# usnistgov/alignn

Measured on NVIDIA H100. Metric: graphs/sec fwd+bwd, higher is better.
Workload: dtype f32

## Files before the change

### alignn_b200/_lib.py

```python
from __future__ import annotations

import ctypes as C
import os
from typing import Optional

import torch

_HERE = os.path.dirname(os.path.abspath(__file__))
LIB_PATH = os.path.join(_HERE, "libalignn_b200.so")

NORM_LAYER, NORM_AFFINE, NORM_STATS = 0, 1, 2
SUPPORTED_D = (32, 64, 128, 256)

_fp = C.c_void_p


class EgcFwdArgs(C.Structure):
    _fields_ = [
        ("struct_size", C.c_size_t),
        ("Nn", C.c_int64), ("Ne", C.c_int64),
        ("d", C.c_int32), ("norm_nodes", C.c_int32), ("norm_edges", C.c_int32), ("residual", C.c_int32),
        ("gate_is_m", C.c_int32),
        ("gate_eps", C.c_float), ("ln_eps", C.c_float),
        ("x", _fp), ("y", _fp), ("G", _fp), ("P", _fp),
        ("src", _fp), ("in_ptr", _fp), ("in_eid", _fp),
        ("n_w", _fp), ("n_b", _fp), ("e_w", _fp), ("e_b", _fp),
        ("x_out", _fp), ("y_out", _fp), ("M", _fp), ("XP", _fp), ("S", _fp), ("H", _fp),
        ("partials", _fp),
        ("stream", _fp),
    ]


class EgcBwdArgs(C.Structure):
    _fields_ = [
        ("struct_size", C.c_size_t),
        ("Nn", C.c_int64), ("Ne", C.c_int64),
        ("d", C.c_int32), ("norm_nodes", C.c_int32), ("norm_edges", C.c_int32),
        ("gate_eps", C.c_float), ("ln_eps", C.c_float),
        ("P", _fp), ("M", _fp), ("XP", _fp), ("S", _fp), ("H", _fp),
        ("src", _fp), ("dst", _fp), ("in_ptr", _fp), ("in_eid", _fp), ("out_ptr", _fp), ("out_eid", _fp),
        ("n_w", _fp), ("n_b", _fp), ("n_mean", _fp), ("n_rstd", _fp),
        ("e_w", _fp), ("e_b", _fp), ("e_mean", _fp), ("e_rstd", _fp),
        ("n_c1", _fp), ("n_c2", _fp), ("e_c1", _fp), ("e_c2", _fp),
        ("gx_out", _fp), ("gy_out", _fp),
        ("GM", _fp), ("GP", _fp), ("GSh", _fp),
        ("partials", _fp), ("partials_src", _fp),
        ("stream", _fp),
    ]


class EgcBwdVjpArgs(C.Structure):
    _fields_ = [
        ("struct_size", C.c_size_t),
        ("Nn", C.c_int64), ("Ne", C.c_int64),
        ("d", C.c_int32), ("norm", C.c_int32),
        ("gate_eps", C.c_float), ("ln_eps", C.c_float),
        ("P", _fp), ("M", _fp), ("XP", _fp), ("S", _fp), ("H", _fp),
        ("src", _fp), ("dst", _fp), ("in_ptr", _fp), ("in_eid", _fp), ("out_ptr", _fp), ("out_eid", _fp),
        ("n_w", _fp), ("n_b", _fp), ("e_w", _fp), ("e_b", _fp),
        ("gx_out", _fp), ("gy_out", _fp), ("GSh", _fp),
        ("GPbar", _fp), ("GMbar", _fp), ("gx_bar_res", _fp), ("gy_bar_res", _fp),
        ("Pbar", _fp), ("Mbar", _fp), ("gx_out_bar", _fp), ("gy_out_bar", _fp), ("Gamma", _fp), ("Shbar", _fp),
        ("partials", _fp), ("partials_src", _fp),
        ("stream", _fp),
    ]


class GemmGatherArgs(C.Structure):
    _fields_ = [
        ("struct_size", C.c_size_t),
        ("M", C.c_int64), ("N", C.c_int32), ("K", C.c_int32),
        ("A", _fp), ("lda", C.c_int64),
        ("w_image", _fp), ("bias", _fp),
        ("add0", _fp), ("ld0", C.c_int64), ("idx0", _fp),
        ("add1", _fp), ("ld1", C.c_int64), ("idx1", _fp),
        ("C", _fp), ("ldc", C.c_int64),
        ("stats", _fp),
        ("stream", _fp),
    ]
# ... 133 lines not shown
```

### alignn_b200/csrc/egc_kernels.cu

```cuda
#include "common.cuh"
#include "api_common.h"
#include "alignn_b200.h"

namespace alignn {

template <int D, bool GIM>
__global__ void __launch_bounds__(kThreads, 2)
egc_forward_kernel(alignn_b200_egc_fwd_args a) {
  using C = RowCfg<D>;
  constexpr int V = C::VPL;
  extern __shared__ __align__(16) float dyn_smem[];
  float* vec = dyn_smem;
  float* sacc = dyn_smem + 4 * D;
  const int lane = threadIdx.x & 31, wib = threadIdx.x >> 5;
  const int64_t warp0 = (int64_t)blockIdx.x * kWarpsPerBlock + wib;
  const int64_t nwarps = (int64_t)gridDim.x * kWarpsPerBlock;
  const bool train = a.XP != nullptr;
  const bool want_res = a.residual && a.y_out && a.norm_edges != ALIGNN_NORM_STATS;
  const bool stats = a.partials != nullptr;
  {
    const float* srcs[4] = {a.n_w, a.n_b, a.e_w, a.e_b};
#pragma unroll
    for (int q = 0; q < 4; ++q)
      for (int i = threadIdx.x; i < D; i += blockDim.x) vec[q * D + i] = srcs[q] ? srcs[q][i] : 0.f;
// ... 369 lines not shown
#pragma unroll
    for (int k = 0; k < V; ++k) t1[k] *= xh[k];
    smem_row_add<D>(acc_gw, t1, lane);
    sa = warp_sum(sa) * (1.f / D);
    sb = warp_sum(sb) * (1.f / D);
#pragma unroll
    for (int k = 0; k < V; ++k) gr[k] = rstd * (gxh[k] - sa - xh[k] * sb);
  } else {
    float mu[V], rs[V], t0[V], t1[V];
    ld_srow<D>(mu, vecs + 2 * D, lane);
    ld_srow<D>(rs, vecs + 3 * D, lane);
#pragma unroll
    for (int k = 0; k < V; ++k) {
      const float gu = go[k] * dsilu_(r[k] * w[k] + b[k]);
      const float xh = (r[k] - mu[k]) * rs[k];
      t0[k] = gu * xh;
      t1[k] = gu;
      gr[k] = w[k] * gu;
      mu[k] = xh;
    }
    smem_row_add<D>(acc_gw, t0, lane);
    smem_row_add<D>(acc_gb, t1, lane);
    if constexpr (mode == ALIGNN_NORM_STATS) {
      float c1[V], c2[V];
      ld_srow<D>(c1, vecs + 4 * D, lane);
      ld_srow<D>(c2, vecs + 5 * D, lane);
#pragma unroll
      for (int k = 0; k < V; ++k) gr[k] -= w[k] * (c1[k] + mu[k] * c2[k]);
    }
  }
}

template <int D, int NORM>
__global__ void __launch_bounds__(kThreads)
egc_backward_dst_kernel(alignn_b200_egc_bwd_args a) {
  using C = RowCfg<D>;
  constexpr int V = C::VPL;
  extern __shared__ __align__(16) float dyn_smem[];
  float* sacc = dyn_smem;
  float* nvec = dyn_smem + kWarpsPerBlock * 6 * D;
  float* sseg = nvec + 12 * D;
  float* evec = nvec + 6 * D;
  {
    const float* srcs[12] = {a.n_w, a.n_b, a.n_mean, a.n_rstd, a.n_c1, a.n_c2, a.e_w, a.e_b, a.e_mean, a.e_rstd, a.e_c1, a.e_c2};
#pragma unroll
    for (int q = 0; q < 12; ++q)
      for (int i = threadIdx.x; i < D; i += blockDim.x) nvec[q * D + i] = srcs[q] ? srcs[q][i] : 0.f;
  }
  __syncthreads();
  const int lane = threadIdx.x & 31, wib = threadIdx.x >> 5;
  const int64_t warp0 = (int64_t)blockIdx.x * kWarpsPerBlock + wib;
  const int64_t nwarps = (int64_t)gridDim.x * kWarpsPerBlock;
  float* acc = sacc + wib * 6 * D;
  for (int i = lane; i < 6 * D; i += 32) acc[i] = 0.f;
  __syncwarp();

  float* wseg = sseg + wib * 2 * D;
  for (int64_t v = warp0; v < a.Nn; v += nwarps) {
    {
      float gsh[V], gs[V];
      float xp[V], go[V], gxp[V], sv[V], hv[V];
      ld_row<D, false>(xp, a.XP + v * D, lane);
      ld_row<D, false>(go, a.gx_out + v * D, lane);
      norm_backward_row<D, NORM>(xp, go, a.ln_eps, nvec, gxp, acc + 2 * D, acc + 3 * D, lane);
      st_row<D, false>(a.GP + v * 4 * D + 3 * D, gxp, lane);
      ld_row<D, false>(sv, a.S + v * D, lane);
      ld_row<D, false>(hv, a.H + v * D, lane);
#pragma unroll
      for (int k = 0; k < V; ++k) {
        const float inv = 1.f / (sv[k] + a.gate_eps);
        gsh[k] = gxp[k] * inv;
        gs[k] = -gxp[k] * hv[k] * inv;
      }
      smem_row_add<D>(acc + 4 * D, gxp, lane);
      st_row<D, false>(a.GSh + v * D, gsh, lane);
      using C2 = RowCfg<D>;
#pragma unroll
      for (int c = 0; c < C2::CH; ++c)
#pragma unroll
        for (int j = 0; j < C2::W; ++j) {
          wseg[c * 32 * C2::W + lane * C2::W + j] = gsh[c * C2::W + j];
          wseg[D + c * 32 * C2::W + lane * C2::W + j] = gs[c * C2::W + j];
        }
      __syncwarp();
    }
    float accB[V];
#pragma unroll
    for (int k = 0; k < V; ++k) accB[k] = 0.f;
    const int p0 = a.in_ptr[v], p1 = a.in_ptr[v + 1];
    for (int base = p0; base < p1; base += 32) {
      const int cnt = min(32, p1 - base);
      int my_e = 0, my_s = 0;
      if (lane < cnt) {
        my_e = a.in_eid ? a.in_eid[base + lane] : base + lane;
        my_s = a.src[my_e];
      }
      float m[V], go[V];
      if (cnt > 0) {
        const int64_t e = __shfl_sync(0xffffffffu, my_e, 0);
        ld_row<D, true>(m, a.M + e * D, lane);
        if (a.gy_out) ld_row<D, true>(go, a.gy_out + e * D, lane);
      }
      for (int i = 0; i < cnt; ++i) {
        const int64_t e = __shfl_sync(0xffffffffu, my_e, i);
        const int64_t s = __shfl_sync(0xffffffffu, my_s, i);
        float cv[V], gm[V], mn[V], gon[V];
        ld_row<D, false>(cv, a.P + s * 4 * D + D, lane);
        const bool more = (i + 1 < cnt);
        if (more) {
          const int64_t en = __shfl_sync(0xffffffffu, my_e, i + 1);
          ld_row<D, true>(mn, a.M + en * D, lane);
          if (a.gy_out) ld_row<D, true>(gon, a.gy_out + en * D, lane);
        }
        if (a.gy_out) {
          norm_backward_row<D, NORM>(m, go, a.ln_eps, evec, gm, acc, acc + D, lane);
        } else {
#pragma unroll
          for (int k = 0; k < V; ++k) gm[k] = 0.f;
        }
        {
          float gsh[V], gs[V];
          ld_srow<D>(gsh, wseg, lane);
          ld_srow<D>(gs, wseg + D, lane);
#pragma unroll
          for (int k = 0; k < V; ++k) {
            const float sg = sigmoidf_(m[k]);
            gm[k] += (gsh[k] * cv[k] + gs[k]) * sg * (1.f - sg);
            accB[k] += gm[k];
          }
        }
        st_row<D, false>(a.GM + e * D, gm, lane);
        if (more) {
#pragma unroll
          for (int k = 0; k < V; ++k) { m[k] = mn[k]; go[k] = gon[k]; }
        }
      }
    }
    st_row<D, false>(a.GP + v * 4 * D + 2 * D, accB, lane);
    smem_row_add<D>(acc + 5 * D, accB, lane);
  }
  __syncthreads();
  if (a.partials) {
    float* out_row = a.partials + (int64_t)blockIdx.x * 6 * D;
    for (int i = threadIdx.x; i < 6 * D; i += blockDim.x) {
      float t = 0.f;
#pragma unroll
      for (int w = 0; w < kWarpsPerBlock; ++w) t += sacc[w * 6 * D + i];
      out_row[i] = t;
    }
  }
}

template <int D>
__global__ void __launch_bounds__(kThreads)
egc_backward_src_kernel(alignn_b200_egc_bwd_args a, float* __restrict__ partials_src, int partial_rows_total) {
  using C = RowCfg<D>;
  constexpr int V = C::VPL;
  __shared__ float red[kWarpsPerBlock * D];
  const int lane = threadIdx.x & 31;
  const int64_t warp0 = (int64_t)blockIdx.x * kWarpsPerBlock + (threadIdx.x >> 5);
  const int64_t nwarps = (int64_t)gridDim.x * kWarpsPerBlock;
  float acc[2][V];
#pragma unroll
  for (int q = 0; q < 2; ++q)
#pragma unroll
    for (int i = 0; i < V; ++i) acc[q][i] = 0.f;

  for (int64_t u = warp0; u < a.Nn; u += nwarps) {
    float accA[V], accC[V];
#pragma unroll
    for (int k = 0; k < V; ++k) { accA[k] = 0.f; accC[k] = 0.f; }
    const int p0 = a.out_ptr[u], p1 = a.out_ptr[u + 1];
    for (int base = p0; base < p1; base += 32) {
      const int cnt = min(32, p1 - base);
      int my_e = 0, my_t = 0;
      if (lane < cnt) {
        my_e = a.out_eid[base + lane];
        my_t = a.dst[my_e];
      }
      int i = 0;
      for (; i + 1 < cnt; i += 2) {
        const int64_t e0 = __shfl_sync(0xffffffffu, my_e, i), t0 = __shfl_sync(0xffffffffu, my_t, i);
        const int64_t e1 = __shfl_sync(0xffffffffu, my_e, i + 1), t1 = __shfl_sync(0xffffffffu, my_t, i + 1);
        float gm0[V], m0[V], gs0[V], gm1[V], m1[V], gs1[V];
        ld_row<D, false>(gm0, a.GM + e0 * D, lane);
        ld_row<D, false>(gm1, a.GM + e1 * D, lane);
        ld_row<D, true>(m0, a.M + e0 * D, lane);
        ld_row<D, true>(m1, a.M + e1 * D, lane);
        ld_row<D, false>(gs0, a.GSh + t0 * D, lane);
        ld_row<D, false>(gs1, a.GSh + t1 * D, lane);
#pragma unroll
        for (int k = 0; k < V; ++k) { accA[k] += gm0[k]; accC[k] += gs0[k] * sigmoidf_(m0[k]); }
#pragma unroll
        for (int k = 0; k < V; ++k) { accA[k] += gm1[k]; accC[k] += gs1[k] * sigmoidf_(m1[k]); }
      }
      if (i < cnt) {
        const int64_t e = __shfl_sync(0xffffffffu, my_e, i);
        const int64_t t = __shfl_sync(0xffffffffu, my_t, i);
        float gm[V], m[V], gsh[V];
        ld_row<D, false>(gm, a.GM + e * D, lane);
        ld_row<D, true>(m, a.M + e * D, lane);
        ld_row<D, false>(gsh, a.GSh + t * D, lane);
#pragma unroll
        for (int k = 0; k < V; ++k) {
          accA[k] += gm[k];
          accC[k] += gsh[k] * sigmoidf_(m[k]);
        }
      }
    }
    st_row<D, false>(a.GP + u * 4 * D, accA, lane);
    st_row<D, false>(a.GP + u * 4 * D + D, accC, lane);
#pragma unroll
    for (int k = 0; k < V; ++k) { acc[0][k] += accA[k]; acc[1][k] += accC[k]; }
  }
  if (partials_src) {
    block_reduce_to_partials<D, 2>(acc, partials_src + (int64_t)blockIdx.x * 2 * D, red);
    const int extra = blockIdx.x + gridDim.x;
    if (extra < partial_rows_total)
      for (int i = threadIdx.x; i < 2 * D; i += blockDim.x) partials_src[(int64_t)extra * 2 * D + i] = 0.f;
  }
}

__global__ void __launch_bounds__(1024)
bn_finalize_kernel(const float* __restrict__ partials, int rows, int stride, int which, double count,
                   int d, const float* __restrict__ gamma, const float* __restrict__ beta, float eps,
                   float momentum, float* running_mean, float* running_var, float* scale, float* shift,
                   float* mean_out, float* rstd_out) {
  __shared__ double ss[32][33], sq[32][33];
  const int cl = threadIdx.x & 31, rl = threadIdx.x >> 5;
  const int c = blockIdx.x * 32 + cl;
  double s = 0.0, q = 0.0;
  if (c < d) {
    const float* p = partials + (size_t)which * 2 * d + c;
    for (int r = rl; r < rows; r += 32) {
      s += (double)p[(size_t)r * stride];
      q += (double)p[(size_t)r * stride + d];
    }
  }
  ss[rl][cl] = s; sq[rl][cl] = q;
  __syncthreads();
  if (rl != 0 || c >= d) return;
#pragma unroll
  for (int k = 1; k < 32; ++k) { s += ss[k][cl]; q += sq[k][cl]; }
  const double mean = s / count;
  double var = q / count - mean * mean;
  if (var < 0.0) var = 0.0;
  const float rstd = (float)(1.0 / sqrt(var + (double)eps));
  const float g = gamma ? gamma[c] : 1.f, b = beta ? beta[c] : 0.f;
  scale[c] = g * rstd;
  shift[c] = b - (float)mean * g * rstd;
  mean_out[c] = (float)mean;
  rstd_out[c] = rstd;
// ... 396 lines not shown
}

int alignn_b200_affine_silu_residual(const float* R, const float* res, const float* scale, const float* shift, float* out,
                                     int64_t n, int d, alignn_stream_t stream) {
  if (!supported_d(d)) return ALIGNN_ERR_UNSUPPORTED_D;
  if (n < 0 || (n > 0 && (!R || !scale || !shift || !out))) return ALIGNN_ERR_BAD_ARG;
  if (n == 0) return ALIGNN_OK;
  const int grid = grid_for_rows(n);
  DISPATCH_D(d, alignn::affine_silu_residual_kernel<D><<<grid, alignn::kThreads, 0, (cudaStream_t)stream>>>(
                    R, res, scale, shift, out, n));
  return check_launch();
}

int alignn_b200_egc_backward(const alignn_b200_egc_bwd_args* a) {
  if (!a) return ALIGNN_ERR_BAD_ARG;
  if (a->struct_size != sizeof(*a)) return ALIGNN_ERR_STRUCT_SIZE;
  if (!supported_d(a->d)) return ALIGNN_ERR_UNSUPPORTED_D;
  if (a->Nn < 0 || a->Ne < 0 || !norm_ok(a->norm_nodes) || !norm_ok(a->norm_edges)) return ALIGNN_ERR_BAD_ARG;
  if (a->Nn == 0) return ALIGNN_OK;
  if (!a->P || !a->XP || !a->S || !a->H || !a->in_ptr || !a->out_ptr || !a->gx_out || !a->GP || !a->GSh ||
      !a->n_w || !a->n_b)
    return ALIGNN_ERR_BAD_ARG;
  if (a->Ne > 0 && (!a->M || !a->src || !a->dst || !a->out_eid || !a->GM)) return ALIGNN_ERR_BAD_ARG;
  if (a->norm_nodes != ALIGNN_NORM_LAYER && (!a->n_mean || !a->n_rstd)) return ALIGNN_ERR_BAD_ARG;
  if (a->norm_nodes == ALIGNN_NORM_STATS && (!a->n_c1 || !a->n_c2)) return ALIGNN_ERR_BAD_ARG;
  if (a->gy_out) {
    if (!a->e_w || !a->e_b) return ALIGNN_ERR_BAD_ARG;
    if (a->norm_edges != ALIGNN_NORM_LAYER && (!a->e_mean || !a->e_rstd)) return ALIGNN_ERR_BAD_ARG;
    if (a->norm_edges == ALIGNN_NORM_STATS && (!a->e_c1 || !a->e_c2)) return ALIGNN_ERR_BAD_ARG;
  }
  cudaStream_t st = (cudaStream_t)a->stream;
  const int grid = grid_for_rows(a->Nn);
  if (a->norm_nodes != a->norm_edges) return ALIGNN_ERR_BAD_ARG;
#define LAUNCH_BWD_DST(NORM)                                                                                   \
  DISPATCH_D(a->d, {                                                                                           \
    const size_t smem_bytes = (size_t)(alignn::kWarpsPerBlock * 8 + 12) * D * sizeof(float);                   \
    static alignn::DeviceOnce configured; int cfg_dev;                                                                            \
    if (configured.needed(&cfg_dev)) {                                                                                         \
      cudaError_t e = cudaFuncSetAttribute(alignn::egc_backward_dst_kernel<D, NORM>,                           \
                                           cudaFuncAttributeMaxDynamicSharedMemorySize, (int)smem_bytes);      \
      if (e != cudaSuccess) return alignn::record_cuda_error((int)e);                                          \
      configured.done(cfg_dev);                                                                                       \
    }                                                                                                          \
    alignn::egc_backward_dst_kernel<D, NORM><<<grid, alignn::kThreads, smem_bytes, st>>>(*a);                  \
  })
  switch (a->norm_nodes) {
    case ALIGNN_NORM_LAYER: LAUNCH_BWD_DST(ALIGNN_NORM_LAYER); break;
    case ALIGNN_NORM_AFFINE: LAUNCH_BWD_DST(ALIGNN_NORM_AFFINE); break;
    default: LAUNCH_BWD_DST(ALIGNN_NORM_STATS); break;
  }
#undef LAUNCH_BWD_DST
  int rc = check_launch();
  if (rc != ALIGNN_OK) return rc;
  DISPATCH_D(a->d, {
    const int grid_src = alignn::one_wave_grid((const void*)alignn::egc_backward_src_kernel<D>, alignn::kThreads, 0, grid);
    if (2 * grid_src < grid) return ALIGNN_ERR_CUDA;
    alignn::egc_backward_src_kernel<D><<<grid_src, alignn::kThreads, 0, st>>>(*a, a->partials_src, grid);
  });
  return check_launch();
}

int alignn_b200_bn_backward_reduce(const float* R, const float* g_out, const float* scale, const float* shift,
                                   const float* mean, const float* rstd, int64_t n, int d, float* partials,
                                   int partial_rows, alignn_stream_t stream) {
  if (!supported_d(d)) return ALIGNN_ERR_UNSUPPORTED_D;
  if (n <= 0 || !R || !g_out || !scale || !shift || !mean || !rstd || !partials) return ALIGNN_ERR_BAD_ARG;
// ... 98 lines not shown
```

### alignn_b200/graph.py

```python
from __future__ import annotations

from typing import Optional, Sequence

import numpy as np
import torch

__all__ = ["Graph", "EdgeIndex", "batch", "unbatch", "reverse", "graph", "as_graph", "bond_cosines"]


def _np(a):
    if isinstance(a, torch.Tensor):
        return a.detach().cpu().numpy()
    return np.asarray(a)


class EdgeIndex:

    __slots__ = ("src", "dst", "in_ptr", "in_eid", "out_ptr", "out_eid", "dst_sorted",
                 "max_in_deg", "num_nodes")

    def __init__(self, src, dst, in_ptr, in_eid, out_ptr, out_eid, dst_sorted, max_in_deg, num_nodes):
        self.src, self.dst = src, dst
        self.in_ptr, self.in_eid = in_ptr, in_eid
        self.out_ptr, self.out_eid = out_ptr, out_eid
        self.dst_sorted = bool(dst_sorted)
        self.max_in_deg = int(max_in_deg)
        self.num_nodes = int(num_nodes)

    @staticmethod
    def build(src: np.ndarray, dst: np.ndarray, num_nodes: int) -> "EdgeIndex":
        from . import _lib
        lib = _lib.load()
        src = np.ascontiguousarray(src, dtype=np.int64).reshape(-1)
        dst = np.ascontiguousarray(dst, dtype=np.int64).reshape(-1)
        E = src.shape[0]
        if E >= 2 ** 31 or num_nodes >= 2 ** 31:
            raise ValueError("graph too large for int32 edge index")
        if dst.shape[0] != E:
            raise ValueError("src and dst differ in length")
        i32 = lambda k: np.empty(k, dtype=np.int32)
        s32, d32, in_ptr, in_eid, out_ptr, out_eid = i32(E), i32(E), i32(num_nodes + 1), i32(E), i32(num_nodes + 1), i32(E)
        flags = np.zeros(2, dtype=np.int32)
        p = lambda a: a.ctypes.data
        rc = lib.alignn_b200_csr_build_host(p(src), p(dst), num_nodes, E, p(s32), p(d32), p(in_ptr), p(in_eid),
                                            p(out_ptr), p(out_eid), p(flags[0:1]), p(flags[1:2]))
        if rc == -1:
            raise ValueError("edge endpoint out of range")
        _lib.check(rc, "alignn_b200_csr_build_host")
        t = torch.from_numpy
        return EdgeIndex(t(s32), t(d32), t(in_ptr), t(in_eid), t(out_ptr), t(out_eid),
                         bool(flags[0]), int(flags[1]), num_nodes)

    @staticmethod
    def build_device(src: torch.Tensor, dst: torch.Tensor, num_nodes: int) -> "EdgeIndex":
        from . import _lib
        lib = _lib.load()
        if not (src.is_cuda and dst.is_cuda):
            raise RuntimeError("EdgeIndex.build_device needs CUDA tensors")
        src = src.to(torch.int32).contiguous()
        dst = dst.to(torch.int32).contiguous()
        E, dev = src.numel(), src.device
        i32 = lambda n: torch.empty(n, device=dev, dtype=torch.int32)
        in_ptr, out_ptr, in_eid, out_eid, flags = i32(num_nodes + 1), i32(num_nodes + 1), i32(E), i32(E), i32(2)
        nb = int(lib.alignn_b200_csr_build_workspace_bytes(num_nodes, E))
        if nb == 0:
            raise ValueError("graph too large for int32 edge index")
        ws = torch.empty(nb, device=dev, dtype=torch.uint8)
        with torch.cuda.device(dev):
            _lib.check(lib.alignn_b200_csr_build(src.data_ptr(), dst.data_ptr(), num_nodes, E, in_ptr.data_ptr(), in_eid.data_ptr(),
                                                 out_ptr.data_ptr(), out_eid.data_ptr(), flags.data_ptr(), ws.data_ptr(), nb,
                                                 _lib.stream_ptr()), "alignn_b200_csr_build")
        f = flags.tolist()
        return EdgeIndex(src, dst, in_ptr, in_eid, out_ptr, out_eid, bool(f[0]), int(f[1]), num_nodes)

    _FIELDS = ("src", "dst", "in_ptr", "in_eid", "out_ptr", "out_eid")

    def to(self, device, non_blocking=False) -> "EdgeIndex":
        moved = [getattr(self, f).to(device, non_blocking=non_blocking) for f in self._FIELDS]
        return EdgeIndex(*moved, self.dst_sorted, self.max_in_deg, self.num_nodes)

    def pin_memory(self) -> "EdgeIndex":
        moved = [getattr(self, f).pin_memory() for f in self._FIELDS]
        return EdgeIndex(*moved, self.dst_sorted, self.max_in_deg, self.num_nodes)

    def nbytes(self) -> int:
        return sum(getattr(self, f).numel() * 4 for f in self._FIELDS)


class _EdgeBatch:

    def __init__(self, g: "Graph"):
        s, d = g.index.src.long(), g.index.dst.long()
        self.src = {k: v[s] for k, v in g.ndata.items()}
        self.dst = {k: v[d] for k, v in g.ndata.items()}
        self.data = dict(g.edata)


class Graph:

    def __init__(self, src=None, dst=None, num_nodes: Optional[int] = None,
                 batch_num_nodes=None, batch_num_edges=None, *, _index: Optional[EdgeIndex] = None):
        if _index is None:
            if isinstance(src, torch.Tensor) and src.is_cuda and num_nodes is not None:
                _index = EdgeIndex.build_device(src.reshape(-1), torch.as_tensor(dst, device=src.device).reshape(-1),
                                                int(num_nodes))
            else:
                src, dst = _np(src).reshape(-1), _np(dst).reshape(-1)
                if num_nodes is None:
                    num_nodes = int(max(src.max(), dst.max())) + 1 if src.size else 0
                _index = EdgeIndex.build(src, dst, int(num_nodes))
        self.index = _index
        self._n = _index.num_nodes
        E = int(_index.src.numel())
        self._bnn = torch.tensor([self._n], dtype=torch.int64) if batch_num_nodes is None \
            else torch.as_tensor(batch_num_nodes, dtype=torch.int64).reshape(-1).cpu()
        self._bne = torch.tensor([E], dtype=torch.int64) if batch_num_edges is None \
            else torch.as_tensor(batch_num_edges, dtype=torch.int64).reshape(-1).cpu()
        if int(self._bnn.sum()) != self._n or int(self._bne.sum()) != E:
            raise ValueError("batch_num_nodes / batch_num_edges do not add up")
# ... 60 lines not shown
            n += sum(v.numel() * v.element_size() for v in d.values())
        return n

    def apply_edges(self, func):
        self.edata.update(func(_EdgeBatch(self)))

    def node_graph_offsets(self) -> torch.Tensor:
        if self._seg.device != self.device:
            self._seg = self._seg.to(self.device)
        return self._seg

    def line_graph(self, backtracking: bool = True, shared: bool = False) -> "Graph":
        if not backtracking:
            raise NotImplementedError("backtracking=False is not used by the reference")
        from . import _lib
        lib = _lib.load()
        ix = self.index
        if self.device.type == "cuda":
            return self._line_graph_device(shared)
        src = np.ascontiguousarray(ix.src.cpu().numpy())
        in_ptr = np.ascontiguousarray(ix.in_ptr.cpu().numpy())
        in_eid = np.ascontiguousarray(ix.in_eid.cpu().numpy())
        E = src.shape[0]
        p = lambda a: a.ctypes.data
        T = int(lib.alignn_b200_line_graph_count_host(p(src), p(in_ptr), p(in_eid), E))
        if T < 0:
            raise RuntimeError("alignn_b200_line_graph_count_host failed")
        li, lj = np.empty(T, dtype=np.int64), np.empty(T, dtype=np.int64)
        bne = np.ascontiguousarray(self._bne.numpy(), dtype=np.int64)
        lbne = np.zeros(bne.shape[0], dtype=np.int64)
        _lib.check(lib.alignn_b200_line_graph_build_host(p(src), p(in_ptr), p(in_eid), E, p(bne), bne.shape[0], T,
                                                         p(li), p(lj), p(lbne)), "alignn_b200_line_graph_build_host")
        lg = Graph(li, lj, E, self._bne.clone(), lbne)
        if self.device.type != "cpu":
            lg = lg.to(self.device)
        if shared:
            lg.ndata.update(self.edata)
        return lg


    def _line_graph_device(self, shared: bool) -> "Graph":
        from . import _lib
        lib = _lib.load()
        ix, dev, E = self.index, self.device, self.num_edges()
        off = torch.empty(E + 1, device=dev, dtype=torch.int32)
        nb = int(lib.alignn_b200_line_graph_workspace_bytes(E))
        ws = torch.empty(max(nb, 1), device=dev, dtype=torch.uint8)
        with torch.cuda.device(dev):
            st = _lib.stream_ptr()
            _lib.check(lib.alignn_b200_line_graph_offsets(ix.src.data_ptr(), ix.dst.data_ptr(), ix.in_ptr.data_ptr(), E,
                                                          off.data_ptr(), ws.data_ptr(), nb, st), "alignn_b200_line_graph_offsets")
            eoff = torch.zeros(self._bne.numel() + 1, dtype=torch.int64)
            eoff[1:] = torch.cumsum(self._bne, 0)
            at = off[eoff.to(dev)].tolist()
            T = int(at[-1])
            lsrc, ldst = (torch.empty(T, device=dev, dtype=torch.int32) for _ in range(2))
            _lib.check(lib.alignn_b200_line_graph_fill(ix.src.data_ptr(), ix.dst.data_ptr(), ix.in_ptr.data_ptr(),
                                                       ix.in_eid.data_ptr(), E, off.data_ptr(), lsrc.data_ptr(), ldst.data_ptr(), st),
                       "alignn_b200_line_graph_fill")
        lbne = torch.tensor([b - a for a, b in zip(at[:-1], at[1:])], dtype=torch.int64)
        lg = Graph(lsrc, ldst, E, self._bne.clone(), lbne)
        if shared:
            lg.ndata.update(self.edata)
        return lg

    def batch_num_nodes_on_device(self) -> torch.Tensor:
        t = getattr(self, "_bnn_dev", None)
        if t is None or t.device != self.device:
            t = self._bnn.to(self.device)
            self._bnn_dev = t
        return t

    def edge_graph_offsets64(self) -> torch.Tensor:
        t = getattr(self, "_eoff64", None)
        if t is None or t.device != self.device:
            t = torch.zeros(self._bne.numel() + 1, dtype=torch.int64)
            t[1:] = torch.cumsum(self._bne, 0)
            t = t.to(self.device)
            self._eoff64 = t
        return t


def graph(data, num_nodes=None) -> Graph:
    return Graph(data[0], data[1], num_nodes)


def batch(graphs: Sequence[Graph]) -> Graph:
    noff, s, d = 0, [], []
    for g in graphs:
        s.append(g.index.src.cpu().numpy().astype(np.int64) + noff)
        d.append(g.index.dst.cpu().numpy().astype(np.int64) + noff)
        noff += g.num_nodes()
    bg = Graph(np.concatenate(s), np.concatenate(d), noff,
               torch.cat([g.batch_num_nodes() for g in graphs]),
# ... 62 lines not shown
```

### alignn_b200/ops.py

```python
from __future__ import annotations

import ctypes as C
import functools
import weakref
from typing import Optional, Tuple

import torch

from . import _lib
from ._lib import NORM_AFFINE, NORM_LAYER, NORM_STATS, ptr, require_cuda, stream_ptr
from .graph import EdgeIndex


def _on_tensor_device(fn):
    @functools.wraps(fn)
    def wrapper(*args, **kw):
        dev = None
        for a in args:
            if isinstance(a, EdgeIndex):
                a = a.src
            elif isinstance(a, (list, tuple)) and a and isinstance(a[0], (list, tuple)) and a[0]:
                a = a[0][0]
            if isinstance(a, torch.Tensor) and a.is_cuda:
                dev = a.device
# ... 138 lines not shown
    partials = torch.empty(rows, 2 * d, device=R.device, dtype=torch.float32)
    with _span("bn_backward_reduce", 8 * n * d):
        _lib.check(lib.alignn_b200_bn_backward_reduce(ptr(R), ptr(g_out), ptr(scale), ptr(shift), ptr(mean), ptr(rstd), n, d,
                                                       ptr(partials), rows, stream_ptr()), "alignn_b200_bn_backward_reduce")
    c = colsum(partials, 1.0 / n)
    return c[:d], c[d:]


@_on_tensor_device
def egc_backward(ix: EdgeIndex, P, M, XP, S, H, gx_out, gy_out, n, e, *, reduce: bool = True, norm_nodes: int, norm_edges: int,
                 gate_eps: float = 1e-6, ln_eps: float = 1e-5, keep_gsh: bool = False):
    lib = _lib.load()
    Nn, d = XP.shape
    Ne = M.shape[0]
    _check_d(d)
    require_cuda(P, M, XP, S, H, gx_out, gy_out, ix.src, ix.dst, ix.in_ptr, ix.in_eid, ix.out_ptr, ix.out_eid,
                 *[t for dct in (n, e) for t in dct.values()])
    dev = XP.device
    new = lambda *s: torch.empty(*s, device=dev, dtype=torch.float32)
    GM, GP, GSh = new(Ne, d), new(Nn, 4 * d), new(Nn, d)
    rows = partial_rows(Nn, d)
    part, part_src = new(rows, 6 * d), new(rows, 2 * d)
    g = lambda dct, k: ptr(dct.get(k))
    a = _lib.EgcBwdArgs(
        struct_size=C.sizeof(_lib.EgcBwdArgs), Nn=Nn, Ne=Ne, d=d, norm_nodes=norm_nodes, norm_edges=norm_edges,
        gate_eps=gate_eps, ln_eps=ln_eps, P=ptr(P), M=ptr(M), XP=ptr(XP), S=ptr(S), H=ptr(H),
        src=ptr(ix.src), dst=ptr(ix.dst), in_ptr=ptr(ix.in_ptr), in_eid=None if ix.dst_sorted else ptr(ix.in_eid),
        out_ptr=ptr(ix.out_ptr), out_eid=ptr(ix.out_eid),
        n_w=g(n, "w"), n_b=g(n, "b"), n_mean=g(n, "mean"), n_rstd=g(n, "rstd"),
        e_w=g(e, "w"), e_b=g(e, "b"), e_mean=g(e, "mean"), e_rstd=g(e, "rstd"),
        n_c1=g(n, "c1"), n_c2=g(n, "c2"), e_c1=g(e, "c1"), e_c2=g(e, "c2"),
        gx_out=ptr(gx_out), gy_out=ptr(gy_out), GM=ptr(GM), GP=ptr(GP), GSh=ptr(GSh),
        partials=ptr(part), partials_src=ptr(part_src), stream=stream_ptr())
    nb = 4 * d * (Ne * (2 + (gy_out is not None)) + 9 * Nn) + 12 * Ne + 4 * d * 2 * Ne
    with _span("egc_backward(dst+src)", nb):
        _lib.check(lib.alignn_b200_egc_backward(C.byref(a)), "alignn_b200_egc_backward")
    extra = (GSh,) if keep_gsh else ()
    if not reduce:
        return (GM, GP, part, part_src) + extra
    return (GM, GP, colsum(part).view(6, d), colsum(part_src).view(2, d)) + extra


@_on_tensor_device
def egc_backward_vjp(ix: EdgeIndex, P, M, XP, S, H, gx_out, gy_out, GSh, GPbar, GMbar, gx_bar_res, gy_bar_res,
                     n_w, n_b, e_w, e_b, *, gate_eps: float = 1e-6, ln_eps: float = 1e-5):
    lib = _lib.load()
    Nn, d = XP.shape
    Ne = M.shape[0]
    _check_d(d)
    require_cuda(P, M, XP, S, H, gx_out, gy_out, GSh, GPbar, GMbar, gx_bar_res, gy_bar_res, n_w, n_b, e_w, e_b,
                 ix.src, ix.dst, ix.in_ptr, ix.in_eid, ix.out_ptr, ix.out_eid)
    dev = XP.device
    new = lambda *s: torch.empty(*s, device=dev, dtype=torch.float32)
    Pbar, Mbar, gxo_bar = new(Nn, 4 * d), new(Ne, d), new(Nn, d)
    gyo_bar = new(Ne, d) if gy_out is not None else None
    Gamma, Shbar = new(Ne, d), new(Nn, d)
    rows = partial_rows(Nn, d)
    part, part_src = new(rows, 6 * d), new(rows, 2 * d)
    a = _lib.EgcBwdVjpArgs(
        struct_size=C.sizeof(_lib.EgcBwdVjpArgs), Nn=Nn, Ne=Ne, d=d, norm=NORM_LAYER, gate_eps=gate_eps, ln_eps=ln_eps,
        P=ptr(P), M=ptr(M), XP=ptr(XP), S=ptr(S), H=ptr(H),
        src=ptr(ix.src), dst=ptr(ix.dst), in_ptr=ptr(ix.in_ptr), in_eid=None if ix.dst_sorted else ptr(ix.in_eid),
        out_ptr=ptr(ix.out_ptr), out_eid=ptr(ix.out_eid),
        n_w=ptr(n_w), n_b=ptr(n_b), e_w=ptr(e_w), e_b=ptr(e_b),
        gx_out=ptr(gx_out), gy_out=ptr(gy_out), GSh=ptr(GSh),
        GPbar=ptr(GPbar), GMbar=ptr(GMbar), gx_bar_res=ptr(gx_bar_res), gy_bar_res=ptr(gy_bar_res),
        Pbar=ptr(Pbar), Mbar=ptr(Mbar), gx_out_bar=ptr(gxo_bar), gy_out_bar=ptr(gyo_bar), Gamma=ptr(Gamma),
        Shbar=ptr(Shbar), partials=ptr(part), partials_src=ptr(part_src), stream=stream_ptr())
# ... 563 lines not shown
```

### alignn_b200/runtime.py

```python
from __future__ import annotations

import math
from typing import Callable, Dict, Tuple

import numpy as np
import torch

from .graph import Graph, batch as batch_graphs, bond_cosines, unbatch


def _star(dT: int) -> Tuple[int, int, int]:
    if dT <= 0:
        return 0, 0, 0
    a = max(1, int(math.isqrt(dT)))
    b = dT // a
    return a, b, dT - a * b


def padding_needs(dE: int, dT: int) -> Tuple[int, int]:
    a, b, r = _star(dT)
    bonds = a + b + ((1 + r) if r else 0)
    return 8, bonds


# ... 51 lines not shown
            if k not in ("atom_features",):
                del p.ndata[k]
    gp = batch_graphs(parts)
    lgp = gp.line_graph(shared=True)
    if lgp.num_edges() != T_b:
        raise RuntimeError(f"padding produced {lgp.num_edges()} bond pairs, wanted {T_b}")
    lgp.edata["h"] = bond_cosines(gp.edata["r"], lgp)
    latp = torch.cat([lat, torch.eye(3, dtype=lat.dtype).unsqueeze(0)], 0)
    return PaddedBatch(gp, lgp, latp, g.batch_size)


class BucketedForward:

    def __init__(self, fn: Callable, device, n_edges, e_edges, t_edges, warmup: int = 2):
        self.fn, self.device = fn, torch.device(device)
        self.n_edges, self.e_edges, self.t_edges = tuple(n_edges), tuple(e_edges), tuple(t_edges)
        self.warmup = warmup
        self._graphs: Dict[tuple, tuple] = {}
        self._stream = torch.cuda.Stream(self.device)

    def bucket(self, g: Graph, lg: Graph) -> tuple:
        N_b = bucket_of(g.num_nodes() + 8, self.n_edges)
        T_b = bucket_of(lg.num_edges(), self.t_edges)
        need_e = padding_needs(0, T_b - lg.num_edges())[1]
        E_b = bucket_of(g.num_edges() + need_e, self.e_edges)
        return N_b, E_b, T_b

    @staticmethod
    def _copy_graph(dst: Graph, src: Graph):
        for f in dst.index._FIELDS:
            getattr(dst.index, f).copy_(getattr(src.index, f), non_blocking=True)
        if dst.index.dst_sorted and not src.index.dst_sorted:
            raise RuntimeError("BucketedForward: line graph of the batch is not destination-sorted")
        dst.index.max_in_deg = src.index.max_in_deg
        dst._seg.copy_(src._seg, non_blocking=True)
        dst._bnn, dst._bne = src._bnn, src._bne
        for name, fresh in (("_bnn_dev", src._bnn), ("_eoff64", None)):
            cached = getattr(dst, name, None)
            if cached is not None:
                if fresh is None:
                    fresh = torch.zeros(src._bne.numel() + 1, dtype=torch.int64)
                    fresh[1:] = torch.cumsum(src._bne, 0)
                cached.copy_(fresh, non_blocking=True)
        for k, v in src.ndata.items():
            dst.ndata[k].copy_(v, non_blocking=True)
        for k, v in src.edata.items():
            dst.edata[k].copy_(v, non_blocking=True)

    def __call__(self, g: Graph, lg: Graph, lat: torch.Tensor):
        key = self.bucket(g, lg)
        pb = pad_batch(g, lg, lat, *key)
        full_key = key + (pb.g.batch_size,)
        entry = self._graphs.get(full_key)
        if entry is None:
            sg, slg, slat = pb.g.to(self.device), pb.lg.to(self.device), pb.lat.to(self.device)
            sg.index.dst_sorted = False
            self._stream.wait_stream(torch.cuda.current_stream(self.device))
            with torch.cuda.stream(self._stream):
                for _ in range(self.warmup):
                    self.fn(sg, slg, slat)
            torch.cuda.current_stream(self.device).wait_stream(self._stream)
            gr = torch.cuda.CUDAGraph()
            with torch.cuda.graph(gr, stream=self._stream):
                out = self.fn(sg, slg, slat)
            entry = (gr, sg, slg, slat, out)
            self._graphs[full_key] = entry
# ... 7 lines not shown
```

### include/alignn_b200.h

```cpp
#ifndef ALIGNN_B200_H
#define ALIGNN_B200_H

#include <stddef.h>
#include <stdint.h>

#ifdef __cplusplus
extern "C" {
#endif

#define ALIGNN_B200_VERSION 101

typedef enum {
  ALIGNN_OK = 0,
  ALIGNN_ERR_BAD_ARG = -1,
  ALIGNN_ERR_UNSUPPORTED_D = -2,
  ALIGNN_ERR_STRUCT_SIZE = -3,
  ALIGNN_ERR_CUDA = -4,
  ALIGNN_ERR_WORKSPACE = -5
} alignn_b200_status;

typedef enum {
  ALIGNN_NORM_LAYER = 0,
  ALIGNN_NORM_AFFINE = 1,
  ALIGNN_NORM_STATS = 2
// ... 36 lines not shown
  alignn_stream_t stream;
} alignn_b200_egc_fwd_args;

int alignn_b200_egc_forward(const alignn_b200_egc_fwd_args* args);

int alignn_b200_bn_finalize(const float* partials, int partial_rows, int partial_stride ,
                            int which ,
                            int64_t count, int d, const float* gamma, const float* beta, float eps, float momentum,
                            float* running_mean, float* running_var ,
                            float* scale, float* shift, float* mean, float* rstd, alignn_stream_t stream);

int alignn_b200_affine_silu_residual(const float* R, const float* res, const float* scale, const float* shift,
                                     float* out, int64_t n, int d, alignn_stream_t stream);

typedef struct {
  size_t struct_size;
  int64_t Nn, Ne;
  int32_t d;
  int32_t norm_nodes, norm_edges;
  float gate_eps, ln_eps;
  const float* P; const float* M; const float* XP; const float* S; const float* H;
  const int32_t* src; const int32_t* dst;
  const int32_t* in_ptr; const int32_t* in_eid;
  const int32_t* out_ptr; const int32_t* out_eid;
  const float* n_w; const float* n_b; const float* n_mean; const float* n_rstd;
  const float* e_w; const float* e_b; const float* e_mean; const float* e_rstd;
  const float* n_c1; const float* n_c2; const float* e_c1; const float* e_c2;
  const float* gx_out;
  const float* gy_out;
  float* GM; float* GP;
  float* GSh;
  float* partials;
  float* partials_src;
  alignn_stream_t stream;
} alignn_b200_egc_bwd_args;

int alignn_b200_egc_backward(const alignn_b200_egc_bwd_args* args);

typedef struct {
  size_t struct_size;
  int64_t Nn, Ne;
  int32_t d;
  int32_t norm;
  float gate_eps, ln_eps;
  const float* P; const float* M; const float* XP; const float* S; const float* H;
  const int32_t* src; const int32_t* dst;
  const int32_t* in_ptr; const int32_t* in_eid;
  const int32_t* out_ptr; const int32_t* out_eid;
  const float* n_w; const float* n_b; const float* e_w; const float* e_b;
  const float* gx_out;
  const float* gy_out;
  const float* GSh;
  const float* GPbar;
  const float* GMbar;
  const float* gx_bar_res;
  const float* gy_bar_res;
  float* Pbar;
  float* Mbar;
  float* gx_out_bar;
  float* gy_out_bar;
  float* Gamma;
  float* Shbar;
  float* partials;
  float* partials_src;
  alignn_stream_t stream;
} alignn_b200_egc_bwd_vjp_args;
// ... 135 lines not shown
```

Before: 4608.

## Add line-graph-aware fused EGC backward kernel using parent graph structure

Result: faster. 4782 (median of 6 runs) (+3.8%).

```diff
diff --git a/alignn_b200/_lib.py b/alignn_b200/_lib.py
--- a/alignn_b200/_lib.py
+++ b/alignn_b200/_lib.py
@@ -45,6 +45,8 @@
         ("gx_out", _fp), ("gy_out", _fp),
         ("GM", _fp), ("GP", _fp), ("GSh", _fp),
         ("partials", _fp), ("partials_src", _fp),
+        ("parent_in_ptr", _fp), ("parent_in_eid", _fp), ("parent_out_ptr", _fp), ("parent_out_eid", _fp),
+        ("parent_Nn", C.c_int64),
         ("stream", _fp),
     ]
 
diff --git a/alignn_b200/csrc/egc_kernels.cu b/alignn_b200/csrc/egc_kernels.cu
--- a/alignn_b200/csrc/egc_kernels.cu
+++ b/alignn_b200/csrc/egc_kernels.cu
@@ -425,6 +425,61 @@
 }
 
 template <int D, int NORM>
+__device__ __forceinline__ void bwd_node_side(const alignn_b200_egc_bwd_args& a, int64_t v, const float* __restrict__ nvec,
+                                              float* __restrict__ acc, float* __restrict__ wseg, int lane) {
+  using C = RowCfg<D>;
+  constexpr int V = C::VPL;
+  float gsh[V], gs[V];
+  float xp[V], go[V], gxp[V], sv[V], hv[V];
+  ld_row<D, false>(xp, a.XP + v * D, lane);
+  ld_row<D, false>(go, a.gx_out + v * D, lane);
+  norm_backward_row<D, NORM>(xp, go, a.ln_eps, nvec, gxp, acc + 2 * D, acc + 3 * D, lane);
+  st_row<D, false>(a.GP + v * 4 * D + 3 * D, gxp, lane);
+  ld_row<D, false>(sv, a.S + v * D, lane);
+  ld_row<D, false>(hv, a.H + v * D, lane);
+#pragma unroll
+  for (int k = 0; k < V; ++k) {
+    const float inv = 1.f / (sv[k] + a.gate_eps);
+    gsh[k] = gxp[k] * inv;
+    gs[k] = -gxp[k] * hv[k] * inv;
+  }
+  smem_row_add<D>(acc + 4 * D, gxp, lane);
+  st_row<D, false>(a.GSh + v * D, gsh, lane);
+#pragma unroll
+  for (int c = 0; c < C::CH; ++c)
+#pragma unroll
+    for (int j = 0; j < C::W; ++j) {
+      wseg[c * 32 * C::W + lane * C::W + j] = gsh[c * C::W + j];
+      wseg[D + c * 32 * C::W + lane * C::W + j] = gs[c * C::W + j];
+    }
+  __syncwarp();
+}
+
+template <int D, int NORM>
+__device__ __forceinline__ void bwd_edge_gm(const alignn_b200_egc_bwd_args& a, const float (&m)[RowCfg<D>::VPL],
+                                           const float (&go)[RowCfg<D>::VPL], const float (&cv)[RowCfg<D>::VPL],
+                                           const float* __restrict__ evec, float* __restrict__ acc,
+                                           const float* __restrict__ wseg, float (&gm)[RowCfg<D>::VPL],
+                                           float (&accB)[RowCfg<D>::VPL], int lane) {
+  constexpr int V = RowCfg<D>::VPL;
+  if (a.gy_out) {
+    norm_backward_row<D, NORM>(m, go, a.ln_eps, evec, gm, acc, acc + D, lane);
+  } else {
+#pragma unroll
+    for (int k = 0; k < V; ++k) gm[k] = 0.f;
+  }
+  float gsh[V], gs[V];
+  ld_srow<D>(gsh, wseg, lane);
+  ld_srow<D>(gs, wseg + D, lane);
+#pragma unroll
+  for (int k = 0; k < V; ++k) {
+    const float sg = sigmoidf_(m[k]);
+    gm[k] += (gsh[k] * cv[k] + gs[k]) * sg * (1.f - sg);
+    accB[k] += gm[k];
+  }
+}
+
+template <int D, int NORM>
 __global__ void __launch_bounds__(kThreads)
 egc_backward_dst_kernel(alignn_b200_egc_bwd_args a) {
   using C = RowCfg<D>;
@@ -450,33 +505,7 @@
 
   float* wseg = sseg + wib * 2 * D;
   for (int64_t v = warp0; v < a.Nn; v += nwarps) {
-    {
-      float gsh[V], gs[V];
-      float xp[V], go[V], gxp[V], sv[V], hv[V];
-      ld_row<D, false>(xp, a.XP + v * D, lane);
-      ld_row<D, false>(go, a.gx_out + v * D, lane);
-      norm_backward_row<D, NORM>(xp, go, a.ln_eps, nvec, gxp, acc + 2 * D, acc + 3 * D, lane);
-      st_row<D, false>(a.GP + v * 4 * D + 3 * D, gxp, lane);
-      ld_row<D, false>(sv, a.S + v * D, lane);
-      ld_row<D, false>(hv, a.H + v * D, lane);
-#pragma unroll
-      for (int k = 0; k < V; ++k) {
-        const float inv = 1.f / (sv[k] + a.gate_eps);
-        gsh[k] = gxp[k] * inv;
-        gs[k] = -gxp[k] * hv[k] * inv;
-      }
-      smem_row_add<D>(acc + 4 * D, gxp, lane);
-      st_row<D, false>(a.GSh + v * D, gsh, lane);
-      using C2 = RowCfg<D>;
-#pragma unroll
-      for (int c = 0; c < C2::CH; ++c)
-#pragma unroll
-        for (int j = 0; j < C2::W; ++j) {
-          wseg[c * 32 * C2::W + lane * C2::W + j] = gsh[c * C2::W + j];
-          wseg[D + c * 32 * C2::W + lane * C2::W + j] = gs[c * C2::W + j];
-        }
-      __syncwarp();
-    }
+    bwd_node_side<D, NORM>(a, v, nvec, acc, wseg, lane);
     float accB[V];
 #pragma unroll
     for (int k = 0; k < V; ++k) accB[k] = 0.f;
@@ -505,23 +534,7 @@
           ld_row<D, true>(mn, a.M + en * D, lane);
           if (a.gy_out) ld_row<D, true>(gon, a.gy_out + en * D, lane);
         }
-        if (a.gy_out) {
-          norm_backward_row<D, NORM>(m, go, a.ln_eps, evec, gm, acc, acc + D, lane);
-        } else {
-#pragma unroll
-          for (int k = 0; k < V; ++k) gm[k] = 0.f;
-        }
-        {
-          float gsh[V], gs[V];
-          ld_srow<D>(gsh, wseg, lane);
-          ld_srow<D>(gs, wseg + D, lane);
-#pragma unroll
-          for (int k = 0; k < V; ++k) {
-            const float sg = sigmoidf_(m[k]);
-            gm[k] += (gsh[k] * cv[k] + gs[k]) * sg * (1.f - sg);
-            accB[k] += gm[k];
-          }
-        }
+        bwd_edge_gm<D, NORM>(a, m, go, cv, evec, acc, wseg, gm, accB, lane);
         st_row<D, false>(a.GM + e * D, gm, lane);
         if (more) {
 #pragma unroll
@@ -583,9 +596,9 @@
         ld_row<D, false>(gs0, a.GSh + t0 * D, lane);
         ld_row<D, false>(gs1, a.GSh + t1 * D, lane);
 #pragma unroll
-        for (int k = 0; k < V; ++k) { accA[k] += gm0[k]; accC[k] += gs0[k] * sigmoidf_(m0[k]); }
-#pragma unroll
-        for (int k = 0; k < V; ++k) { accA[k] += gm1[k]; accC[k] += gs1[k] * sigmoidf_(m1[k]); }
+        for (int k = 0; k < V; ++k) { accA[k] += gm0[k]; accC[k] = fmaf(gs0[k], sigmoidf_(m0[k]), accC[k]); }
+#pragma unroll
+        for (int k = 0; k < V; ++k) { accA[k] += gm1[k]; accC[k] = fmaf(gs1[k], sigmoidf_(m1[k]), accC[k]); }
       }
       if (i < cnt) {
         const int64_t e = __shfl_sync(0xffffffffu, my_e, i);
@@ -597,7 +610,7 @@
 #pragma unroll
         for (int k = 0; k < V; ++k) {
           accA[k] += gm[k];
-          accC[k] += gsh[k] * sigmoidf_(m[k]);
+          accC[k] = fmaf(gsh[k], sigmoidf_(m[k]), accC[k]);
         }
       }
     }
@@ -611,6 +624,173 @@
     const int extra = blockIdx.x + gridDim.x;
     if (extra < partial_rows_total)
       for (int i = threadIdx.x; i < 2 * D; i += blockDim.x) partials_src[(int64_t)extra * 2 * D + i] = 0.f;
+  }
+}
+
+constexpr int kLineWarps = 12;
+constexpr int kLineThreads = kLineWarps * 32;
+
+template <int D>
+constexpr size_t line_bwd_smem_floats() {
+  return (size_t)(kLineWarps * 6 + 12 + kLineWarps * 2 + 2 * kLineWarps * 2 + 2) * D;
+}
+
+template <int D, int NORM>
+__global__ void __launch_bounds__(kLineThreads, 1)
+egc_backward_line_kernel(alignn_b200_egc_bwd_args a, int partial_rows_total) {
+  using C = RowCfg<D>;
+  constexpr int V = C::VPL;
+  constexpr int W = kLineWarps;
+  extern __shared__ __align__(16) float dyn_smem[];
+  float* sacc = dyn_smem;
+  float* nvec = sacc + W * 6 * D;
+  float* evec = nvec + 6 * D;
+  float* sseg = nvec + 12 * D;
+  float* stage = sseg + W * 2 * D;
+  float* ssrc = stage + 2 * W * 2 * D;
+  __shared__ int sself[W];
+  {
+    const float* srcs[12] = {a.n_w, a.n_b, a.n_mean, a.n_rstd, a.n_c1, a.n_c2, a.e_w, a.e_b, a.e_mean, a.e_rstd, a.e_c1, a.e_c2};
+#pragma unroll
+    for (int q = 0; q < 12; ++q)
+      for (int i = threadIdx.x; i < D; i += blockDim.x) nvec[q * D + i] = srcs[q] ? srcs[q][i] : 0.f;
+  }
+  for (int i = threadIdx.x; i < W * 6 * D; i += blockDim.x) sacc[i] = 0.f;
+  for (int i = threadIdx.x; i < 2 * D; i += blockDim.x) ssrc[i] = 0.f;
+  const int lane = threadIdx.x & 31, wib = threadIdx.x >> 5;
+  float* acc = sacc + wib * 6 * D;
+  float* wseg = sseg + wib * 2 * D;
+  int round = 0;
+
+  for (int64_t at = blockIdx.x; at < a.parent_Nn; at += gridDim.x) {
+    const int ip0 = a.parent_in_ptr[at], kin = a.parent_in_ptr[at + 1] - ip0;
+    const int op0 = a.parent_out_ptr[at], kout = a.parent_out_ptr[at + 1] - op0;
+    if (kout == 0) {
+      for (int t = 0; t < kin; ++t) {
+        const int64_t i = a.parent_in_eid[ip0 + t];
+        for (int q = threadIdx.x; q < 2 * D; q += blockDim.x) a.GP[i * 4 * D + q] = 0.f;
+      }
+      continue;
+    }
+    for (int c0 = 0; c0 < kout; c0 += W) {
+      const int nd = min(W, kout - c0);
+      const bool last_chunk = c0 + W >= kout;
+      const bool active = wib < nd;
+      __syncthreads();
+      int64_t j = 0, ebase = 0;
+      int selfpos = -1;
+      if (active) {
+        j = a.parent_out_eid[op0 + c0 + wib];
+        ebase = a.in_ptr[j];
+        if (a.in_ptr[j + 1] - ebase != kin) {
+          for (int t0 = 0; t0 < kin; t0 += 32) {
+            const bool hit = t0 + lane < kin && a.parent_in_eid[ip0 + t0 + lane] == (int)j;
+            const unsigned bal = __ballot_sync(0xffffffffu, hit);
+            if (bal) { selfpos = t0 + __ffs(bal) - 1; break; }
+          }
+        }
+        if (lane == 0) sself[wib] = selfpos;
+        bwd_node_side<D, NORM>(a, j, nvec, acc, wseg, lane);
+      }
+      auto edge_of = [&](int t) { return ebase + t - ((selfpos >= 0 && t > selfpos) ? 1 : 0); };
+      const int my_i = lane < kin ? a.parent_in_eid[ip0 + lane] : 0;
+      auto source = [&](int t) { return t < 32 ? __shfl_sync(0xffffffffu, my_i, t) : a.parent_in_eid[ip0 + t]; };
+      float accB[V], m[V], go[V], cv[V];
+#pragma unroll
+      for (int k = 0; k < V; ++k) accB[k] = 0.f;
+      int tn = selfpos == 0 ? 1 : 0;
+      {
+        const int64_t in_ = kin > 0 ? source(min(tn, kin - 1)) : 0;
+        if (active && tn < kin) {
+          const int64_t e = edge_of(tn);
+          ld_row<D, true>(m, a.M + e * D, lane);
+          if (a.gy_out) ld_row<D, true>(go, a.gy_out + e * D, lane);
+          ld_row<D, false>(cv, a.P + in_ * 4 * D + D, lane);
+        }
+      }
+      const int q = threadIdx.x * 4;
+      static_assert(2 * D <= 4 * kLineThreads, "one float4 of GP[i, 0:2d] per thread");
+      for (int t = 0; t < kin; ++t, ++round) {
+        const int64_t i = source(t);
+        float* stg = stage + (round & 1) * W * 2 * D;
+        float4 r = make_float4(0.f, 0.f, 0.f, 0.f);
+        if (c0 > 0 && q < 2 * D) r = *reinterpret_cast<const float4*>(a.GP + i * 4 * D + q);
+        const int tnext = (t + 1 == selfpos) ? t + 2 : t + 1;
+        const int64_t inext = source(min(tnext, kin - 1));
+        if (active && t != selfpos) {
+          const int64_t e = edge_of(t);
+          float gm[V], mn[V], gon[V], cvn[V];
+          if (tnext < kin) {
+            const int64_t en = edge_of(tnext);
+            ld_row<D, true>(mn, a.M + en * D, lane);
+            if (a.gy_out) ld_row<D, true>(gon, a.gy_out + en * D, lane);
+            ld_row<D, false>(cvn, a.P + inext * 4 * D + D, lane);
+          }
+          bwd_edge_gm<D, NORM>(a, m, go, cv, evec, acc, wseg, gm, accB, lane);
+          st_row<D, false>(a.GM + e * D, gm, lane);
+          float sg[V];
+#pragma unroll
+          for (int k = 0; k < V; ++k) sg[k] = sigmoidf_(m[k]);
+#pragma unroll
+          for (int c = 0; c < C::CH; ++c)
+#pragma unroll
+            for (int u = 0; u < C::W; ++u) {
+              stg[wib * 2 * D + c * 32 * C::W + lane * C::W + u] = gm[c * C::W + u];
+              stg[wib * 2 * D + D + c * 32 * C::W + lane * C::W + u] = sg[c * C::W + u];
+            }
+          if (tnext < kin) {
+#pragma unroll
+            for (int k = 0; k < V; ++k) { m[k] = mn[k]; go[k] = gon[k]; cv[k] = cvn[k]; }
+          }
+        }
+        __syncthreads();
+        if (q < 2 * D) {
+          if (q < D) {
+            for (int w = 0; w < nd; ++w) {
+              if (t == sself[w]) continue;
+              const float4 g = *reinterpret_cast<const float4*>(stg + w * 2 * D + q);
+              r.x += g.x; r.y += g.y; r.z += g.z; r.w += g.w;
+            }
+          } else {
+            for (int w = 0; w < nd; ++w) {
+              if (t == sself[w]) continue;
+              const float4 g = *reinterpret_cast<const float4*>(sseg + w * 2 * D + (q - D));
+              const float4 sg = *reinterpret_cast<const float4*>(stg + w * 2 * D + q);
+              r.x = fmaf(g.x, sg.x, r.x); r.y = fmaf(g.y, sg.y, r.y); r.z = fmaf(g.z, sg.z, r.z); r.w = fmaf(g.w, sg.w, r.w);
+            }
+          }
+          *reinterpret_cast<float4*>(a.GP + i * 4 * D + q) = r;
+          if (last_chunk) {
+            float4* s4 = reinterpret_cast<float4*>(ssrc + q);
+            float4 u = *s4;
+            u.x += r.x; u.y += r.y; u.z += r.z; u.w += r.w;
+            *s4 = u;
+          }
+        }
+      }
+      if (active) {
+        st_row<D, false>(a.GP + j * 4 * D + 2 * D, accB, lane);
+        smem_row_add<D>(acc + 5 * D, accB, lane);
+      }
+    }
+  }
+  __syncthreads();
+  if (a.partials) {
+    float* out_row = a.partials + (int64_t)blockIdx.x * 6 * D;
+    for (int i = threadIdx.x; i < 6 * D; i += blockDim.x) {
+      float t = 0.f;
+#pragma unroll
+      for (int w = 0; w < W; ++w) t += sacc[w * 6 * D + i];
+      out_row[i] = t;
+    }
+  }
+  if (a.partials_src)
+    for (int i = threadIdx.x; i < 2 * D; i += blockDim.x) a.partials_src[(int64_t)blockIdx.x * 2 * D + i] = ssrc[i];
+  for (int64_t r = blockIdx.x + gridDim.x; r < partial_rows_total; r += gridDim.x) {
+    if (a.partials)
+      for (int i = threadIdx.x; i < 6 * D; i += blockDim.x) a.partials[r * 6 * D + i] = 0.f;
+    if (a.partials_src)
+      for (int i = threadIdx.x; i < 2 * D; i += blockDim.x) a.partials_src[r * 2 * D + i] = 0.f;
   }
 }
 
@@ -1073,6 +1253,34 @@
   cudaStream_t st = (cudaStream_t)a->stream;
   const int grid = grid_for_rows(a->Nn);
   if (a->norm_nodes != a->norm_edges) return ALIGNN_ERR_BAD_ARG;
+  const bool line = a->parent_in_ptr || a->parent_in_eid || a->parent_out_ptr || a->parent_out_eid || a->parent_Nn;
+  if (line) {
+    if (!a->parent_in_ptr || !a->parent_out_ptr || a->parent_Nn <= 0 ||
+        (a->Nn > 0 && (!a->parent_in_eid || !a->parent_out_eid)) || (a->Ne > 0 && (!a->M || !a->GM)))
+      return ALIGNN_ERR_BAD_ARG;
+#define LAUNCH_BWD_LINE(NORM)                                                                                   \
+  DISPATCH_D(a->d, {                                                                                           \
+    const size_t smem_bytes = alignn::line_bwd_smem_floats<D>() * sizeof(float);                               \
+    static alignn::DeviceOnce configured; int cfg_dev;                                                         \
+    if (configured.needed(&cfg_dev)) {                                                                         \
+      cudaError_t e = cudaFuncSetAttribute(alignn::egc_backward_line_kernel<D, NORM>,                          \
+                                           cudaFuncAttributeMaxDynamicSharedMemorySize, (int)smem_bytes);      \
+      if (e != cudaSuccess) return alignn::record_cuda_error((int)e);                                          \
+      configured.done(cfg_dev);                                                                                \
+    }                                                                                                          \
+    const int64_t want = a->parent_Nn < grid ? a->parent_Nn : grid;                                            \
+    const int grid_line = alignn::one_wave_grid((const void*)alignn::egc_backward_line_kernel<D, NORM>,        \
+                                                alignn::kLineThreads, smem_bytes, (int)want);                  \
+    alignn::egc_backward_line_kernel<D, NORM><<<grid_line, alignn::kLineThreads, smem_bytes, st>>>(*a, grid);  \
+  })
+    switch (a->norm_nodes) {
+      case ALIGNN_NORM_LAYER: LAUNCH_BWD_LINE(ALIGNN_NORM_LAYER); break;
+      case ALIGNN_NORM_AFFINE: LAUNCH_BWD_LINE(ALIGNN_NORM_AFFINE); break;
+      default: LAUNCH_BWD_LINE(ALIGNN_NORM_STATS); break;
+    }
+#undef LAUNCH_BWD_LINE
+    return check_launch();
+  }
 #define LAUNCH_BWD_DST(NORM)                                                                                   \
   DISPATCH_D(a->d, {                                                                                           \
     const size_t smem_bytes = (size_t)(alignn::kWarpsPerBlock * 8 + 12) * D * sizeof(float);                   \
diff --git a/alignn_b200/graph.py b/alignn_b200/graph.py
--- a/alignn_b200/graph.py
+++ b/alignn_b200/graph.py
@@ -17,15 +17,16 @@
 class EdgeIndex:
 
     __slots__ = ("src", "dst", "in_ptr", "in_eid", "out_ptr", "out_eid", "dst_sorted",
-                 "max_in_deg", "num_nodes")
-
-    def __init__(self, src, dst, in_ptr, in_eid, out_ptr, out_eid, dst_sorted, max_in_deg, num_nodes):
+                 "max_in_deg", "num_nodes", "parent")
+
+    def __init__(self, src, dst, in_ptr, in_eid, out_ptr, out_eid, dst_sorted, max_in_deg, num_nodes, parent=None):
         self.src, self.dst = src, dst
         self.in_ptr, self.in_eid = in_ptr, in_eid
         self.out_ptr, self.out_eid = out_ptr, out_eid
         self.dst_sorted = bool(dst_sorted)
         self.max_in_deg = int(max_in_deg)
         self.num_nodes = int(num_nodes)
+        self.parent = None if parent is None else tuple(parent)
 
     @staticmethod
     def build(src: np.ndarray, dst: np.ndarray, num_nodes: int) -> "EdgeIndex":
@@ -77,14 +78,17 @@
 
     def to(self, device, non_blocking=False) -> "EdgeIndex":
         moved = [getattr(self, f).to(device, non_blocking=non_blocking) for f in self._FIELDS]
-        return EdgeIndex(*moved, self.dst_sorted, self.max_in_deg, self.num_nodes)
+        parent = None if self.parent is None else [t.to(device, non_blocking=non_blocking) for t in self.parent]
+        return EdgeIndex(*moved, self.dst_sorted, self.max_in_deg, self.num_nodes, parent)
 
     def pin_memory(self) -> "EdgeIndex":
         moved = [getattr(self, f).pin_memory() for f in self._FIELDS]
-        return EdgeIndex(*moved, self.dst_sorted, self.max_in_deg, self.num_nodes)
+        parent = None if self.parent is None else [t.pin_memory() for t in self.parent]
+        return EdgeIndex(*moved, self.dst_sorted, self.max_in_deg, self.num_nodes, parent)
 
     def nbytes(self) -> int:
-        return sum(getattr(self, f).numel() * 4 for f in self._FIELDS)
+        n = sum(getattr(self, f).numel() * 4 for f in self._FIELDS)
+        return n + (0 if self.parent is None else sum(t.numel() * 4 for t in self.parent))
 
 
 class _EdgeBatch:
@@ -211,6 +215,7 @@
         _lib.check(lib.alignn_b200_line_graph_build_host(p(src), p(in_ptr), p(in_eid), E, p(bne), bne.shape[0], T,
                                                          p(li), p(lj), p(lbne)), "alignn_b200_line_graph_build_host")
         lg = Graph(li, lj, E, self._bne.clone(), lbne)
+        lg.index.parent = (ix.in_ptr, ix.in_eid, ix.out_ptr, ix.out_eid)
         if self.device.type != "cpu":
             lg = lg.to(self.device)
         if shared:
@@ -239,6 +244,7 @@
                        "alignn_b200_line_graph_fill")
         lbne = torch.tensor([b - a for a, b in zip(at[:-1], at[1:])], dtype=torch.int64)
         lg = Graph(lsrc, ldst, E, self._bne.clone(), lbne)
+        lg.index.parent = (ix.in_ptr, ix.in_eid, ix.out_ptr, ix.out_eid)
         if shared:
             lg.ndata.update(self.edata)
         return lg
diff --git a/alignn_b200/ops.py b/alignn_b200/ops.py
--- a/alignn_b200/ops.py
+++ b/alignn_b200/ops.py
@@ -194,8 +194,17 @@
         n_c1=g(n, "c1"), n_c2=g(n, "c2"), e_c1=g(e, "c1"), e_c2=g(e, "c2"),
         gx_out=ptr(gx_out), gy_out=ptr(gy_out), GM=ptr(GM), GP=ptr(GP), GSh=ptr(GSh),
         partials=ptr(part), partials_src=ptr(part_src), stream=stream_ptr())
-    nb = 4 * d * (Ne * (2 + (gy_out is not None)) + 9 * Nn) + 12 * Ne + 4 * d * 2 * Ne
-    with _span("egc_backward(dst+src)", nb):
+    if ix.parent is not None:
+        pin, peid, pout, poeid = ix.parent
+        require_cuda(pin, peid, pout, poeid)
+        a.parent_in_ptr, a.parent_in_eid, a.parent_out_ptr, a.parent_out_eid = ptr(pin), ptr(peid), ptr(pout), ptr(poeid)
+        a.parent_Nn = pin.numel() - 1
+        name = "egc_backward(line)"
+        nb = 4 * d * (Ne * (2 + (gy_out is not None)) + 10 * Nn) + 4 * (2 * pin.numel() + 2 * Nn + Nn + 1)
+    else:
+        name = "egc_backward(dst+src)"
+        nb = 4 * d * (Ne * (2 + (gy_out is not None)) + 9 * Nn) + 12 * Ne + 4 * d * 2 * Ne
+    with _span(name, nb):
         _lib.check(lib.alignn_b200_egc_backward(C.byref(a)), "alignn_b200_egc_backward")
     extra = (GSh,) if keep_gsh else ()
     if not reduce:
diff --git a/alignn_b200/runtime.py b/alignn_b200/runtime.py
--- a/alignn_b200/runtime.py
+++ b/alignn_b200/runtime.py
@@ -107,6 +107,10 @@
             getattr(dst.index, f).copy_(getattr(src.index, f), non_blocking=True)
         if dst.index.dst_sorted and not src.index.dst_sorted:
             raise RuntimeError("BucketedForward: line graph of the batch is not destination-sorted")
+        if (dst.index.parent is None) != (src.index.parent is None):
+            raise RuntimeError("BucketedForward: line-graph descriptor present in only one of the batches")
+        for t, u in zip(dst.index.parent or (), src.index.parent or ()):
+            t.copy_(u, non_blocking=True)
         dst.index.max_in_deg = src.index.max_in_deg
         dst._seg.copy_(src._seg, non_blocking=True)
         dst._bnn, dst._bne = src._bnn, src._bne
diff --git a/include/alignn_b200.h b/include/alignn_b200.h
--- a/include/alignn_b200.h
+++ b/include/alignn_b200.h
@@ -92,6 +92,9 @@
   float* GSh;
   float* partials;
   float* partials_src;
+  const int32_t* parent_in_ptr; const int32_t* parent_in_eid;
+  const int32_t* parent_out_ptr; const int32_t* parent_out_eid;
+  int64_t parent_Nn;
   alignn_stream_t stream;
 } alignn_b200_egc_bwd_args;
 
```
